# mobeets/classifying-vae-lstm

Hardware: AMD Instinct MI355X
Metric: piano-roll timesteps/sec (train) (higher is better)
Workload: dtype f32; 1 GPU; cfg3: cl_vrnn batch 256/GPU x seq_len 128, latent 2, 10 classes, 88-dim piano-roll, Adam-WN, hipGraph=True; global_batch=256, seq_len=128, parallelism=dp1

## Files before the change

### classifying-vae-lstm_amd/csrc/label_head.hip

```cpp
#include "common.h"
#include "lstm_pair_pack.h"
#include "philox.h"
#include "reduce_job.h"
#include "label_bwd_row.h"

namespace clv {

struct LabelFwdArgs {
  int B, D, C, G4;
  const float* hW;
  __device__ float* hW_out() const { return const_cast<float*>(hW); }
  const float* Ka;
  const float* ba;
  float* eps;
  struct { int on; uint32_t k0, k1, stream, step; uint64_t first; const int32_t* step_dev; } noise;
  const float* onehot;
  float prior;
  const float* Kenc_w;
  const float* benc;
  const float* Kdec_w;
  const float* bdec;
  float* wargs;
  float* W;
  float* rowloss;
  float* rb_enc;
  float* rb_dec;
};

template <int NT>
__device__ __forceinline__ void label_fwd_row(const LabelFwdArgs& a, int b, int tid, const float* s_h, float* s_wargs, float* s_w,
                                              long long oh_row = -1) {
  const int C1 = a.C - 1, NA = 2 * C1;
  __shared__ float s_eps[LH_MAXC], s_oh[LH_MAXC];
  if (tid >= NT - 64 && tid - (NT - 64) < a.C) {
    const int j = tid - (NT - 64);
    float e = 0.f;
    if (j < C1) {
      if (a.noise.on) {
        e = philox_normal_at(a.noise.first + (uint64_t)b * C1 + j, a.noise.k0, a.noise.k1, a.noise.stream,
                             a.noise.step + (a.noise.step_dev ? (uint32_t)*a.noise.step_dev : 0u));
        a.eps[(size_t)b * C1 + j] = e;
      } else {
        e = a.eps[(size_t)b * C1 + j];
      }
    }
    s_eps[j] = e;
    s_oh[j] = a.onehot ? a.onehot[(size_t)(oh_row < 0 ? b : oh_row) * a.C + j] : 0.f;
  }
  {
    __shared__ float s_part[16][2 * LH_MAXC];
    constexpr int KSL = NT / 64 < 16 ? NT / 64 : 16;
    const int col = tid & 63, sl = tid >> 6;
    if (sl < KSL) {
      float kv[(128 + KSL - 1) / KSL];
      const int cc = min(col, NA - 1);
#pragma unroll
      for (int i = 0; i < (128 + KSL - 1) / KSL; ++i) kv[i] = a.Ka[(size_t)min(sl + KSL * i, a.D - 1) * NA + cc];
      float acc = 0.f;
#pragma unroll
      for (int i = 0; i < (128 + KSL - 1) / KSL; ++i) acc = fmaf(sl + KSL * i < a.D ? s_h[sl + KSL * i] : 0.f, kv[i], acc);
      if (col < NA) s_part[sl][col] = acc;
    }
    __syncthreads();
    if (tid < NA) {
      float acc = a.ba[tid];
#pragma unroll
      for (int i = 0; i < KSL; ++i) acc += s_part[i][tid];
      s_wargs[tid] = acc;
      a.wargs[(size_t)b * NA + tid] = acc;
    }
  }
  __syncthreads();
  if (tid == 0) {
    float e[LH_MAXC];
    float S = 1.f, klw = 0.f;
    const float ep = __expf(a.prior);
    for (int j = 0; j < C1; ++j) {
      const float m = s_wargs[j], lv = s_wargs[C1 + j];
      const float sd = expf(0.5f * lv);
      e[j] = expf(m + sd * s_eps[j]);
      S += e[j];
      klw += 1.f - a.prior + lv - sd * sd / ep - m * m / ep;
    }
    e[C1] = 1.f;
    const float invS = 1.f / S;
    float qs = 0.f, wbest = -1.f, tbest = -1.f;
    int amax = 0, tmax = 0;
    for (int j = 0; j < a.C; ++j) {
      const float w = e[j] * invS;
      s_w[j] = w;
      a.W[(size_t)b * a.C + j] = w;
      qs += w + LW2;
      if (w > wbest) { wbest = w; amax = j; }
      const float tj = s_oh[j];
      if (tj > tbest) { tbest = tj; tmax = j; }
    }
    float wrec = 0.f;
    if (a.onehot)
      for (int j = 0; j < a.C; ++j) {
        const float n = (s_w[j] + LW2) / qs;
        wrec -= s_oh[j] * logf(fminf(fmaxf(n, LEPS_K), 1.f - LEPS_K));
      }
    a.rowloss[(size_t)b * 3 + 0] = -0.5f * klw;
    a.rowloss[(size_t)b * 3 + 1] = (float)C1 * wrec;
    a.rowloss[(size_t)b * 3 + 2] = (a.onehot && amax == tmax) ? 1.f : 0.f;
  }
  __syncthreads();
  for (int c = tid; c < a.G4; c += NT) {
    float e = a.benc[c], d = a.bdec[c];
    for (int j0 = 0; j0 < a.C; j0 += 8) {
      float ke[8], kd[8];
#pragma unroll
      for (int q = 0; q < 8; ++q) {
        const int j = min(j0 + q, a.C - 1);
        ke[q] = a.Kenc_w[(size_t)j * a.G4 + c];
        kd[q] = a.Kdec_w[(size_t)j * a.G4 + c];
      }
#pragma unroll
      for (int q = 0; q < 8; ++q) {
        const float w = j0 + q < a.C ? s_w[j0 + q] : 0.f;
        e = fmaf(w, ke[q], e);
        d = fmaf(w, kd[q], d);
      }
    }
    a.rb_enc[(size_t)b * a.G4 + c] = e;
    a.rb_dec[(size_t)b * a.G4 + c] = d;
  }
}

__global__ __launch_bounds__(LH_T) void vrnn_label_fwd_kernel(LabelFwdArgs a) {
  __shared__ float s_h[128], s_wargs[2 * LH_MAXC], s_w[LH_MAXC];
  const int b = blockIdx.x, tid = threadIdx.x;
  if (tid < a.D) s_h[tid] = a.hW[(size_t)b * a.D + tid];
  __syncthreads();
  label_fwd_row<LH_T>(a, b, tid, s_h, s_wargs, s_w);
}

struct LabelFwdXArgs {
  LabelFwdArgs l;
  const float* X;
  const float* Kh;
  const float* bh;
  int nx, ldx;
  PairPackArgs pack;
  const float* part; int splits;
  struct Stage {
    int on;
    const unsigned char* cur; const unsigned char* hist;
    long long cur_stride, cur_offset, hist_stride, hist_offset, row0;
    const long long* cur_table; const long long* hist_table; const long long* idx;
    const int* step_dev; int step0, period; long long cur_s, cur_o;
    float* X; float* Xh; int hist_chunk; long long hist_ld;
    const float* w_src; float* w_out;
    unsigned char* X8; unsigned char* Xh8;
  } stage;
};
__device__ __forceinline__ void label_fwd_x_block(const LabelFwdXArgs& ax, const int b, float2 (*part)[64], float* s_h, float* s_wargs,
                                                  float* s_w) {
  const LabelFwdArgs& a = ax.l;
  const int tid = threadIdx.x, lane = tid & 63;
  if (ax.pack.out) {
    for (int i = b * 1024 + tid; i < PK_TOTAL; i += a.B * 1024)
      ax.pack.out[i] = pair_pack_element(i, ax.pack.L, ax.pack.U_e, ax.pack.U_d, ax.pack.Kz, ax.pack.Wz,
                                         [](const float* p) { return *p; });
  }
  const int wave = __builtin_amdgcn_readfirstlane(tid >> 6);
  const int n2 = a.D / 2;
  const int lc = min(lane, n2 - 1);
  const float2* K2 = reinterpret_cast<const float2*>(ax.Kh);
  const float* xr = ax.X + (size_t)b * ax.ldx;
  const unsigned char* xbytes = nullptr;
  long long oh_row = -1;
  if (ax.stage.on) {
    const LabelFwdXArgs::Stage& g = ax.stage;
    long long base = 0;
    if (g.step_dev) {
      int j = (*g.step_dev - g.step0) % g.period;
      j = j < 0 ? j + g.period : j;
      base = (long long)j * g.cur_s + g.cur_o;
    }
    const long long sr = g.idx ? g.idx[base + b] : g.row0 + base + b;
    oh_row = sr;
    xbytes = g.cur + (g.cur_table ? g.cur_table[sr] : sr) * g.cur_stride + g.cur_offset;
    const unsigned char* hb = g.hist ? g.hist + (g.hist_table ? g.hist_table[sr] : sr) * g.hist_stride + g.hist_offset : nullptr;
    if (g.X8) {
      unsigned* xo8 = reinterpret_cast<unsigned*>(g.X8 + (size_t)b * ax.nx);
      unsigned* ho8 = reinterpret_cast<unsigned*>(g.Xh8 + (size_t)b * ax.nx);
      for (int c = 4 * tid; c < ax.nx; c += 4 * 1024) {
        xo8[c >> 2] = *reinterpret_cast<const unsigned*>(xbytes + c);
        if (hb) ho8[c >> 2] = *reinterpret_cast<const unsigned*>(hb + c);
      }
    } else {
      float* xo = g.X + (size_t)b * ax.ldx;
      for (int c = 4 * tid; c < ax.nx; c += 4 * 1024) {
        const unsigned v = *reinterpret_cast<const unsigned*>(xbytes + c);
        *reinterpret_cast<float4*>(xo + c) = make_float4((float)(v & 255u), (float)((v >> 8) & 255u), (float)((v >> 16) & 255u), (float)(v >> 24));
      }
      if (hb) {
        const int pieces = ax.nx / g.hist_chunk;
        for (int c = 4 * tid; c < ax.nx; c += 4 * 1024) {
          const unsigned v = *reinterpret_cast<const unsigned*>(hb + c);
          const int p = c / g.hist_chunk, w = c - p * g.hist_chunk;
          *reinterpret_cast<float4*>(g.Xh + ((size_t)b * pieces + p) * g.hist_ld + w) =
              make_float4((float)(v & 255u), (float)((v >> 8) & 255u), (float)((v >> 16) & 255u), (float)(v >> 24));
        }
      }
    }
    if (g.w_out && tid < a.C) g.w_out[(size_t)b * a.C + tid] = g.w_src[(size_t)sr * a.C + tid];
  }
  float2 acc = make_float2(0.f, 0.f);
  const int nchunk = (ax.nx + 63) / 64;
  typedef const __attribute__((address_space(1))) unsigned* gwords;
  auto xload = [&](int ch) -> unsigned {
    const int i = min(min(ch, nchunk - 1) * 64 + lane, ax.nx - 1);
    return xbytes ? ((gwords)xbytes)[i >> 2] : __builtin_bit_cast(unsigned, xr[i]);
  };
  const int xsh = 8 * (lane & 3);
  auto xval = [&](unsigned raw) { return xbytes ? (float)((raw >> xsh) & 0xffu) : __builtin_bit_cast(float, raw); };
  unsigned xa = xload(wave), xb = xload(wave + 16);
  for (int ch = wave; ch < nchunk; ch += 32) {
    const float x0 = xval(xa), x1 = xval(xb);
    const int j0 = ch * 64, j1 = (ch + 16) * 64;
    xa = xload(ch + 32); xb = xload(ch + 48);
    unsigned long long m0 = __ballot(j0 + lane < ax.nx && x0 != 0.f);
    unsigned long long m1 = __ballot(ch + 16 < nchunk && j1 + lane < ax.nx && x1 != 0.f);
    while (m0 | m1) {
      int kk[8];
      float vv[8];
#pragma unroll
      for (int q = 0; q < 8; ++q) {
        unsigned long long& m = q < 4 ? m0 : m1;
        const bool on = m != 0;
        const int bit = on ? __builtin_ctzll(m) : 0;
        m = on ? (m & (m - 1)) : 0;
        kk[q] = (q < 4 ? j0 : j1) + bit;
        const float v = __builtin_bit_cast(float, __builtin_amdgcn_readlane(__builtin_bit_cast(int, q < 4 ? x0 : x1), bit));
        vv[q] = on ? v : 0.f;
      }
      float2 kr[8];
#pragma unroll
      for (int q = 0; q < 8; ++q) kr[q] = K2[(size_t)min(kk[q], ax.nx - 1) * n2 + lc];
#pragma unroll
      for (int q = 0; q < 8; ++q) { acc.x = fmaf(vv[q], kr[q].x, acc.x); acc.y = fmaf(vv[q], kr[q].y, acc.y); }
    }
  }
  part[wave][lane] = acc;
  __syncthreads();
  if (wave == 0 && lane < n2) {
    float2 t = make_float2(ax.bh[2 * lane], ax.bh[2 * lane + 1]);
#pragma unroll
    for (int w = 0; w < 16; ++w) { t.x += part[w][lane].x; t.y += part[w][lane].y; }
    t.x = fmaxf(t.x, 0.f); t.y = fmaxf(t.y, 0.f);
    s_h[2 * lane] = t.x; s_h[2 * lane + 1] = t.y;
    float* op = a.hW_out() + (size_t)b * a.D + 2 * lane;
    op[0] = t.x; op[1] = t.y;
  }
  __syncthreads();
  label_fwd_row<1024>(a, b, tid, s_h, s_wargs, s_w, oh_row);
}

__global__ __launch_bounds__(1024) void vrnn_label_fwd_x_kernel(LabelFwdXArgs ax) {
  __shared__ float2 part[16][64];
  __shared__ float s_h[128], s_wargs[2 * LH_MAXC], s_w[LH_MAXC];
  label_fwd_x_block(ax, (int)blockIdx.x, part, s_h, s_wargs, s_w);
}

constexpr int FP_RMAX = 64;
constexpr int FP_NC = 4;
#ifndef FP_PF
#define FP_PF 4
#endif
#ifndef FP_ROUND
#define FP_ROUND 1
#endif
#ifndef FP_ABL
#define FP_ABL 0
#endif
typedef unsigned u32x4_t __attribute__((ext_vector_type(4)));
struct FrameProjArgs {
  int T, N, ldo, wgs, nset;
  const float* K[2];
  float* out[2];
};

#ifdef FRONT_STAMPS
__device__ unsigned long long g_front_wg[2048][6];
#define FRONT_STAMP(k)                                                                                               \
  do {                                                                                                               \
    __syncthreads();                                                                                                 \
    if (threadIdx.x == 0 && blockIdx.x < 2048) {                                                                     \
      unsigned long long t__;                                                                                        \
      unsigned hw__, xcc__;                                                                                          \
      asm volatile("s_memrealtime %0\n\ts_waitcnt lgkmcnt(0)" : "=s"(t__));                                          \
      asm volatile("s_getreg_b32 %0, hwreg(HW_REG_HW_ID)" : "=s"(hw__));                                             \
      asm volatile("s_getreg_b32 %0, hwreg(HW_REG_XCC_ID)" : "=s"(xcc__));                                           \
      g_front_wg[blockIdx.x][k < 2 ? k : k + 2] = t__;                                                                \
      g_front_wg[blockIdx.x][2] = hw__; g_front_wg[blockIdx.x][3] = xcc__;                                           \
    }                                                                                                                \
  } while (0)
#else
#define FRONT_STAMP(k)
#endif

__device__ __forceinline__ void frame_proj_block(const LabelFwdXArgs& ax, const FrameProjArgs& fp, const int u, float* Kl,
                                                 const unsigned char** rowp) {
  const LabelFwdXArgs::Stage& g = ax.stage;
  const int tid = threadIdx.x, lane = tid & 63;
  const int wave = __builtin_amdgcn_readfirstlane(tid >> 6);
  const int grp = u / fp.wgs, w = u - grp * fp.wgs;
  const bool second = grp >= 2;
  const int nf = ax.l.D, B = ax.l.B;
  const int nch = fp.N / 2, c0 = (grp & 1) * nch;
  const float* K = second ? fp.K[1] : fp.K[0];
  float* out = second ? fp.out[1] : fp.out[0];
  {
    const int q4 = nch / 4, nv = nf * q4;
    float4* dst = reinterpret_cast<float4*>(Kl);
    for (int i0 = tid; i0 < nv; i0 += 4 * 1024) {
      float4 v[4];
#pragma unroll
      for (int q = 0; q < 4; ++q) {
        const int e = min(i0 + q * 1024, nv - 1), k = e / q4;
        v[q] = *reinterpret_cast<const float4*>(K + (size_t)k * fp.N + c0 + 4 * (e - k * q4));
      }
#pragma unroll
      for (int q = 0; q < 4; ++q)
        if (i0 + q * 1024 < nv) dst[i0 + q * 1024] = v[q];
    }
  }
  const int nrows = w < B ? (B - w + fp.wgs - 1) / fp.wgs : 0;
  if (tid < nrows) {
    const int b = w + tid * fp.wgs;
    long long base = 0;
    if (g.step_dev) {
      int j = (*g.step_dev - g.step0) % g.period;
      j = j < 0 ? j + g.period : j;
      base = (long long)j * g.cur_s + g.cur_o;
    }
    const long long sr = g.idx ? g.idx[base + b] : g.row0 + base + b;
    rowp[tid] = second ? g.hist + (g.hist_table ? g.hist_table[sr] : sr) * g.hist_stride + g.hist_offset
                       : g.cur + (g.cur_table ? g.cur_table[sr] : sr) * g.cur_stride + g.cur_offset;
  }
  __syncthreads();
  FRONT_STAMP(2);
  const int nq = nrows * fp.T;
  if (nq == 0) return;
  const int colb = min(lane, nch / 4 - 1) * 4;
  const unsigned vo = lane < nch / 4 ? (unsigned)lane * 16u : 0x80000000u;
  const __amdgpu_buffer_rsrc_t r_out = __builtin_amdgcn_make_buffer_rsrc(out, 0, (int)((size_t)B * fp.T * fp.ldo * 4), 0x00020000);
  const int k0 = min(lane, nf - 1), k1 = min(lane + 64, nf - 1);
  const bool v0 = lane < nf, v1 = lane + 64 < nf;
  typedef const __attribute__((address_space(1))) unsigned* gwords;
  const int w0 = k0 >> 2, w1 = k1 >> 2, sh0 = 8 * (k0 & 3), sh1 = 8 * (k1 & 3), nfw = nf / 4;
  auto rowbase = [&](int r) -> gwords {
    const unsigned long long p = (unsigned long long)rowp[min(r, nrows - 1)];
    const unsigned lo = __builtin_amdgcn_readfirstlane((unsigned)p), hi = __builtin_amdgcn_readfirstlane((unsigned)(p >> 32));
    return (gwords)(((unsigned long long)hi << 32) | lo);
  };
  const gwords base0 = rowbase(0);
  auto frame = [&](gwords base, int t, unsigned& x0, unsigned& x1) {
    gwords bp = base + t * nfw;
    x0 = bp[w0]; x1 = bp[w1];
  };
  int ri = wave / fp.T, t = wave - ri * fp.T;
  int ra = ri, ta = t;
  gwords base_a = rowbase(ra);
  auto advance_a = [&]() {
    ta += 16;
    if (ta >= fp.T) {
      do { ta -= fp.T; ++ra; } while (ta >= fp.T);
      base_a = rowbase(ra);
    }
  };
  const unsigned so_step = 16u * (unsigned)fp.ldo * 4u, so_wrap = (unsigned)(fp.wgs - 1) * (unsigned)fp.T * (unsigned)fp.ldo * 4u;
  unsigned so = (unsigned)(((w + ri * fp.wgs) * fp.T + t) * fp.ldo + c0) * 4u;
  auto advance_c = [&]() {
    t += 16; so += so_step;
    while (t >= fp.T) { t -= fp.T; so += so_wrap; }
  };
  unsigned qx0[FP_PF], qx1[FP_PF];
#pragma unroll
  for (int j = 0; j < FP_PF; ++j) {
    const bool ok = wave + 16 * j < nq;
    frame(ok ? base_a : base0, ok ? ta : 0, qx0[j], qx1[j]);
    __builtin_amdgcn_raw_buffer_store_b128(u32x4_t{0u, 0u, 0u, 0u}, r_out, (int)0x80000000u, 0, 0);
    advance_a();
  }
  for (int qb = wave; qb < nq; qb += 16 * FP_PF) {
#pragma unroll
    for (int j = 0; j < FP_PF; ++j) {
      const int q = qb + 16 * j;
      const bool live = q < nq;
      const float fx0 = (float)((qx0[j] >> sh0) & 0xffu), fx1 = (float)((qx1[j] >> sh1) & 0xffu);
      const bool more = q + 16 * FP_PF < nq;
      if (FP_ABL != 3) frame(more ? base_a : base0, more ? ta : 0, qx0[j], qx1[j]);
      advance_a();
      unsigned long long m0 = __ballot(live && v0 && fx0 != 0.f), m1 = __ballot(live && v1 && fx1 != 0.f);
      float acc[FP_NC];
#pragma unroll
      for (int c = 0; c < FP_NC; ++c) acc[c] = 0.f;
      auto rounds = [&](unsigned long long m, const float fx, const int kbase) {
        if (FP_ROUND == 1) {
          while (m) {
            const int k = __builtin_ctzll(m);
            asm("s_bitset0_b64 %0, %1" : "+s"(m) : "s"(k));
            const float v = __builtin_bit_cast(float, __builtin_amdgcn_readlane(__builtin_bit_cast(int, fx), k));
            const float4 k4 = *reinterpret_cast<const float4*>(Kl + (kbase + k) * nch + colb);
            acc[0] = fmaf(v, k4.x, acc[0]); acc[1] = fmaf(v, k4.y, acc[1]); acc[2] = fmaf(v, k4.z, acc[2]); acc[3] = fmaf(v, k4.w, acc[3]);
          }
          return;
        }
        while (m) {
          float v[FP_ROUND], kv[FP_ROUND][FP_NC];
          bool on[FP_ROUND];
#pragma unroll
          for (int r = 0; r < FP_ROUND; ++r) {
            on[r] = m != 0;
            const int k = on[r] ? __builtin_ctzll(m) : 0;
            m &= m - 1;
            v[r] = __builtin_bit_cast(float, __builtin_amdgcn_readlane(__builtin_bit_cast(int, fx), k));
            const float4 k4 = *reinterpret_cast<const float4*>(Kl + (kbase + k) * nch + colb);
            kv[r][0] = k4.x; kv[r][1] = k4.y; kv[r][2] = k4.z; kv[r][3] = k4.w;
          }
#pragma unroll
          for (int r = 0; r < FP_ROUND; ++r)
#pragma unroll
            for (int c = 0; c < FP_NC; ++c) acc[c] = (r == 0 || on[r]) ? fmaf(v[r], kv[r][c], acc[c]) : acc[c];
        }
      };
      if (FP_ABL != 2) {
        rounds(m0, fx0, 0);
        rounds(m1, fx1, 64);
      } else {
        acc[0] = fx0; acc[1] = fx1;
      }
      __builtin_amdgcn_raw_buffer_store_b128(u32x4_t{__builtin_bit_cast(unsigned, acc[0]), __builtin_bit_cast(unsigned, acc[1]),
                                                      __builtin_bit_cast(unsigned, acc[2]), __builtin_bit_cast(unsigned, acc[3])},
                                             r_out, (int)((live && FP_ABL != 1) ? vo : 0x80000000u), (int)so, 0);
      advance_c();
    }
  }
}

__global__ __launch_bounds__(1024) __attribute__((amdgpu_num_sgpr(72))) void vrnn_front_kernel(LabelFwdXArgs ax, FrameProjArgs fp) {
  __shared__ float2 part[16][64];
  __shared__ float s_h[128], s_wargs[2 * LH_MAXC], s_w[LH_MAXC];
  __shared__ const unsigned char* rowp[FP_RMAX];
  extern __shared__ __attribute__((aligned(16))) float fp_kl[];
  FRONT_STAMP(0);
  if ((int)blockIdx.x < ax.l.B) label_fwd_x_block(ax, (int)blockIdx.x, part, s_h, s_wargs, s_w);
  else frame_proj_block(ax, fp, (int)blockIdx.x - ax.l.B, fp_kl, rowp);
  FRONT_STAMP(1);
}

__global__ __launch_bounds__(LH_T) void vrnn_label_fwd_parts_kernel(LabelFwdXArgs ax) {
  constexpr int NWV = LH_T / 64;
  __shared__ float2 part[NWV][64];
  __shared__ float s_h[128], s_wargs[2 * LH_MAXC], s_w[LH_MAXC];
  const LabelFwdArgs& a = ax.l;
  const int tid = threadIdx.x, lane = tid & 63;
  if (ax.pack.out) {
    for (int i = blockIdx.x * LH_T + tid; i < PK_TOTAL; i += gridDim.x * LH_T)
      ax.pack.out[i] = pair_pack_element(i, ax.pack.L, ax.pack.U_e, ax.pack.U_d, ax.pack.Kz, ax.pack.Wz,
                                         [](const float* p) { return *p; });
  }
  const int wave = __builtin_amdgcn_readfirstlane(tid >> 6);
  const int b = blockIdx.x;
  const int n2 = a.D / 2;
  const int lc = min(lane, n2 - 1);
  float2 acc = make_float2(0.f, 0.f);
  const float2* pp = reinterpret_cast<const float2*>(ax.part + (size_t)b * a.D) + lc;
  const size_t cs = (size_t)a.B * a.D / 2;
  for (int c0 = wave; c0 < ax.splits; c0 += 8 * NWV) {
    float2 v[8];
#pragma unroll
    for (int q = 0; q < 8; ++q) v[q] = pp[(size_t)min(c0 + NWV * q, ax.splits - 1) * cs];
#pragma unroll
    for (int q = 0; q < 8; ++q) {
      const float mk = c0 + NWV * q < ax.splits ? 1.f : 0.f;
      acc.x = fmaf(v[q].x, mk, acc.x); acc.y = fmaf(v[q].y, mk, acc.y);
    }
  }
  part[wave][lane] = acc;
  __syncthreads();
  if (wave == 0 && lane < n2) {
    float2 t = make_float2(ax.bh[2 * lane], ax.bh[2 * lane + 1]);
#pragma unroll
    for (int w = 0; w < NWV; ++w) { t.x += part[w][lane].x; t.y += part[w][lane].y; }
    t.x = fmaxf(t.x, 0.f); t.y = fmaxf(t.y, 0.f);
    s_h[2 * lane] = t.x; s_h[2 * lane + 1] = t.y;
    float* op = a.hW_out() + (size_t)b * a.D + 2 * lane;
    op[0] = t.x; op[1] = t.y;
  }
  __syncthreads();
  label_fwd_row<LH_T>(a, b, tid, s_h, s_wargs, s_w);
}

__global__ __launch_bounds__(LH_T) void vrnn_label_bwd_kernel(LabelBwdArgs a) {
  label_bwd_row<LH_T>(a, (int)blockIdx.x, (int)threadIdx.x);
}

}

using namespace clv;

extern "C" int clv_vrnn_label_fwd(int B, int D, int C, int G4, const float* hW, const float* Ka, const float* ba,
                                  const float* eps, const float* onehot, float prior_logvar,
                                  const float* Kenc_w, const float* benc, const float* Kdec_w, const float* bdec,
                                  float* wargs, float* W, float* rowloss, float* rb_enc, float* rb_dec, void* stream) {
  if (B <= 0 || D <= 0 || D > 128 || C < 2 || C > LH_MAXC || G4 <= 0) return CLV_EINVAL;
  if (!hW || !Ka || !ba || !eps || !Kenc_w || !benc || !Kdec_w || !bdec || !wargs || !W || !rowloss || !rb_enc || !rb_dec)
    return CLV_EINVAL;
  LabelFwdArgs a{B, D, C, G4, hW, Ka, ba, const_cast<float*>(eps), {0, 0, 0, 0, 0, 0, nullptr}, onehot, prior_logvar, Kenc_w, benc,
                 Kdec_w, bdec, wargs, W, rowloss, rb_enc, rb_dec};
  hipStream_t s = (hipStream_t)stream;
  ProfScope p("vrnn_label_fwd", s);
  hipLaunchKernelGGL(vrnn_label_fwd_kernel, dim3(B), dim3(LH_T), 0, s, a);
  return launch_status();
}

extern "C" size_t clv_vrnn_label_bwd_workspace_bytes(int B, int D, int C) {
  return (size_t)B * (D + 1) * 2 * (C - 1) * sizeof(float);
}

extern "C" int clv_vrnn_label_bwd(int B, int D, int C, int G4, const float* dzsum_enc, const float* dzsum_dec,
                                     const float* Kenc_w, const float* Kdec_w, const float* wargs, const float* eps,
                                     const float* onehot, const float* W, const float* hW, const float* Ka,
                                     float prior_logvar, float class_weight, float w_kl_weight, float inv_b,
                                     float* dwargs, float* dhW, float* dKa, float* dba, void* ws, size_t ws_bytes,
                                     clv_reduce_job* job, void* stream) {
  if (job) memset(job, 0, sizeof(*job));
  if (B <= 0 || D <= 0 || D > 128 || C < 2 || C > LH_MAXC || G4 <= 0) return CLV_EINVAL;
  if (!dzsum_enc || !dzsum_dec || !Kenc_w || !Kdec_w || !wargs || !eps || !onehot || !W || !hW || !Ka || !dwargs || !dhW)
    return CLV_EINVAL;
  const bool wg = dKa != nullptr;
  if (wg && (!dba || !ws || ws_bytes < clv_vrnn_label_bwd_workspace_bytes(B, D, C))) return CLV_EWORKSPACE;
  LabelBwdArgs a{B, D, C, G4, dzsum_enc, dzsum_dec, Kenc_w, Kdec_w, wargs, eps, onehot, W, hW, Ka,
                 prior_logvar, class_weight, w_kl_weight, inv_b, dwargs, dhW, wg ? (float*)ws : nullptr};
  hipStream_t s = (hipStream_t)stream;
  {
    ProfScope p("vrnn_label_bwd", s);
    hipLaunchKernelGGL(vrnn_label_bwd_kernel, dim3(B), dim3(LH_T), 0, s, a);
  }
  int st = launch_status();
  if (st || !wg) return st;
  ReduceJob j;
  memset(&j, 0, sizeof(j));
  const int NA = 2 * (C - 1);
  j.partial = (const float*)ws;
  j.M = D + 1; j.N = NA; j.splits = B; j.nprob = 2;
  j.alpha = 1.f; j.beta = 0.f; j.act = CLV_ACT_NONE;
  j.prob[0] = ReduceProb{dKa, NA, 0};
  j.prob[1] = ReduceProb{dba, NA, D};
  if (job && B > 1) memcpy(job, &j, sizeof(j));
  else st = launch_reduce(j, s);
  return st;
}

extern "C" int clv_vrnn_label_fwd_x_proj_supported(int B, int D, int nx, int T, int N);

static int label_fwd_x_launch(int B, int D, int C, int G4, const float* X, int ldx, int nx, const float* Kh, const float* part,
                              int splits, const clv_label_stage* stage, const float* bh, float* hW_out, const float* Ka, const float* ba,
                              float* eps, const float* onehot, float prior_logvar,
                              const float* Kenc_w, const float* benc, const float* Kdec_w, const float* bdec,
                              float* wargs, float* W, float* rowloss, float* rb_enc, float* rb_dec,
                              const clv_noise_draw* noise, const clv_pair_pack_src* pack, const clv_frame_proj* proj, void* stream) {
  if (pack && (pack->H != LH || !clv_lstm_pair_supported(pack->H, pack->L) || !pack->U_enc || !pack->U_dec || !pack->Kz ||
               !pack->Wz || !pack->pack || ((uintptr_t)pack->pack) % 16))
    return CLV_EINVAL;
  if (B <= 0 || D <= 0 || D > 128 || D % 2 != 0 || C < 2 || C > LH_MAXC || G4 <= 0) return CLV_EINVAL;
  if (part ? (splits <= 0 || ((uintptr_t)part) % 8 != 0)
           : (nx <= 0 || ldx < nx || (!X && !(stage && stage->X8)) || !Kh || ((uintptr_t)Kh) % 8 != 0)) return CLV_EINVAL;
  if (stage) {
    const clv_label_stage& g = *stage;
    if (part || !g.cur || nx % 4 || ldx % 4 || ((uintptr_t)g.cur) % 4 || g.cur_stride % 4 || g.cur_offset % 4) return CLV_EINVAL;
    if (g.hist && (((uintptr_t)g.hist) % 4 || g.hist_stride % 4 || g.hist_offset % 4)) return CLV_EINVAL;
    if (g.X8) {
      if (((uintptr_t)g.X8) % 4 || (g.hist && (!g.Xh8 || ((uintptr_t)g.Xh8) % 4))) return CLV_EINVAL;
    } else {
      if (!g.X || ((uintptr_t)g.X) % 16) return CLV_EINVAL;
      if (g.hist && (!g.Xh || g.hist_chunk <= 0 || g.hist_chunk % 4 || nx % g.hist_chunk || g.hist_ld % 4 || g.hist_ld < g.hist_chunk ||
                     ((uintptr_t)g.Xh) % 16))
        return CLV_EINVAL;
    }
    if ((g.w_out != nullptr) != (g.w_src != nullptr)) return CLV_EINVAL;
    if (g.cursor.step_dev && g.cursor.period < 1) return CLV_EINVAL;
  }
  if (!bh || !hW_out || !Ka || !ba || !eps || !Kenc_w || !benc || !Kdec_w || !bdec || !wargs || !W || !rowloss ||
      !rb_enc || !rb_dec)
    return CLV_EINVAL;
  LabelFwdXArgs a{{B, D, C, G4, hW_out, Ka, ba, eps, {0, 0, 0, 0, 0, 0, nullptr}, onehot, prior_logvar, Kenc_w, benc, Kdec_w, bdec,
                   wargs, W, rowloss, rb_enc, rb_dec}, X, Kh, bh, nx, ldx, {0, nullptr, nullptr, nullptr, nullptr, nullptr}, part, splits, {}};
  if (stage) {
    const clv_label_stage& g = *stage;
    a.stage = LabelFwdXArgs::Stage{1, g.cur, g.hist, (long long)g.cur_stride, (long long)g.cur_offset, (long long)g.hist_stride,
                                   (long long)g.hist_offset, (long long)g.row0, (const long long*)g.cur_table,
                                   (const long long*)g.hist_table, (const long long*)g.idx, g.cursor.step_dev, g.cursor.step0,
                                   g.cursor.period, (long long)g.cursor.stride, (long long)g.cursor.offset, g.X, g.Xh, g.hist_chunk,
                                   (long long)g.hist_ld, g.w_src, g.w_out, g.X8, g.Xh8};
    if (g.w_src) a.l.onehot = g.w_src;
  }
  if (pack) a.pack = PairPackArgs{pack->L, pack->U_enc, pack->U_dec, pack->Kz, pack->Wz, reinterpret_cast<float4*>(pack->pack)};
  if (noise) {
    a.l.noise.on = 1; a.l.noise.k0 = (uint32_t)noise->seed; a.l.noise.k1 = (uint32_t)(noise->seed >> 32);
    a.l.noise.stream = noise->stream; a.l.noise.step = noise->step; a.l.noise.first = noise->first;
    a.l.noise.step_dev = noise->step_dev;
  }
  hipStream_t s = (hipStream_t)stream;
  if (proj) {
    if (!clv_vrnn_label_fwd_x_proj_supported(B, D, nx, proj->T, proj->N) || !stage || !stage->X8 || part || proj->ldo < proj->N ||
        (size_t)B * proj->T * proj->ldo * 4 >= ((size_t)1 << 31) || proj->ldo % 4 || ((uintptr_t)proj->out_cur) % 16 || ((uintptr_t)proj->out_hist) % 16 ||
        !proj->K_cur || !proj->out_cur || ((uintptr_t)proj->K_cur) % 16 || (proj->K_hist && (!proj->out_hist || !stage->hist ||
        ((uintptr_t)proj->K_hist) % 16)))
      return CLV_EINVAL;
    FrameProjArgs fp;
    memset(&fp, 0, sizeof(fp));
    fp.T = proj->T; fp.N = proj->N; fp.ldo = proj->ldo; fp.nset = proj->K_hist ? 2 : 1;
    fp.K[0] = proj->K_cur; fp.out[0] = proj->out_cur; fp.K[1] = proj->K_hist; fp.out[1] = proj->out_hist;
    const int groups = 2 * fp.nset;
    int wgs = 256 / groups;
    wgs = wgs > B ? B : wgs;
    const int need = (B + FP_RMAX - 1) / FP_RMAX;
    wgs = wgs < need ? need : wgs;
    fp.wgs = wgs;
    size_t lds = (size_t)D * (proj->N / 2) * sizeof(float);
#ifdef FRONT_STAMPS
    if (const char* e = getenv("CLV_EXP_FRONT_LDS")) lds = (size_t)atoi(e);
#endif
    if (int e = clv::allow_dynamic_lds(reinterpret_cast<const void*>(vrnn_front_kernel), 64 * 1024)) return e;
    ProfScope p("vrnn_front", s);
    hipLaunchKernelGGL(vrnn_front_kernel, dim3(B + groups * wgs), dim3(1024), lds, s, a, fp);
    return launch_status();
  }
  ProfScope p("vrnn_label_fwd", s);
  if (part) hipLaunchKernelGGL(vrnn_label_fwd_parts_kernel, dim3(B), dim3(LH_T), 0, s, a);
  else hipLaunchKernelGGL(vrnn_label_fwd_x_kernel, dim3(B), dim3(1024), 0, s, a);
  return launch_status();
}

#ifdef FRONT_STAMPS
extern "C" int clv_debug_front_wg(unsigned long long* host_out) {
  return (int)hipMemcpyFromSymbol(host_out, HIP_SYMBOL(clv::g_front_wg), sizeof(unsigned long long) * 2048 * 6);
}
#endif

extern "C" int clv_vrnn_label_fwd_x_proj_supported(int B, int D, int nx, int T, int N) {
  return B >= 1 && D >= 4 && D <= 128 && D % 4 == 0 && T >= 1 && (long long)T * D == nx && N >= 8 && N % 8 == 0 && N / 2 <= 64 * clv::FP_NC &&
         (size_t)D * (N / 2) * sizeof(float) <= 64 * 1024 && (size_t)B * T * N * sizeof(float) < ((size_t)1 << 31);
}

extern "C" int clv_vrnn_label_fwd_x(int B, int D, int C, int G4, const float* X, int ldx, int nx, const float* Kh,
                                    const clv_label_stage* stage,
                                    const float* bh, float* hW_out, const float* Ka, const float* ba,
                                    float* eps, const float* onehot, float prior_logvar,
                                    const float* Kenc_w, const float* benc, const float* Kdec_w, const float* bdec,
                                    float* wargs, float* W, float* rowloss, float* rb_enc, float* rb_dec,
                                    const clv_noise_draw* noise, const clv_pair_pack_src* pack, const clv_frame_proj* proj,
                                    void* stream) {
  if (stage)
    return label_fwd_x_launch(B, D, C, G4, stage->X, ldx, nx, Kh, nullptr, 0, stage, bh, hW_out, Ka, ba, eps, stage->w_src,
                              prior_logvar, Kenc_w, benc, Kdec_w, bdec, wargs, W, rowloss, rb_enc, rb_dec, noise, pack, proj, stream);
  if (proj) return CLV_EINVAL;
  return label_fwd_x_launch(B, D, C, G4, X, ldx, nx, Kh, nullptr, 0, nullptr, bh, hW_out, Ka, ba, eps, onehot, prior_logvar, Kenc_w, benc,
                            Kdec_w, bdec, wargs, W, rowloss, rb_enc, rb_dec, noise, pack, nullptr, stream);
}

extern "C" int clv_vrnn_label_fwd_parts(int B, int D, int C, int G4, const float* part, int splits,
                                        const float* bh, float* hW_out, const float* Ka, const float* ba,
                                        float* eps, const float* onehot, float prior_logvar,
                                        const float* Kenc_w, const float* benc, const float* Kdec_w, const float* bdec,
                                        float* wargs, float* W, float* rowloss, float* rb_enc, float* rb_dec,
                                        const clv_noise_draw* noise, const clv_pair_pack_src* pack, void* stream) {
  if (!part) return CLV_EINVAL;
  return label_fwd_x_launch(B, D, C, G4, nullptr, 0, 0, nullptr, part, splits, nullptr, bh, hW_out, Ka, ba, eps, onehot, prior_logvar, Kenc_w,
                            benc, Kdec_w, bdec, wargs, W, rowloss, rb_enc, rb_dec, noise, pack, nullptr, stream);
}
```

Measured before the change: 101.5 million timesteps/s.

## Restructure sparse frame projection into per-quarter-wave nonzero compaction via LDS lists

Rewrites the piano-roll frame-projection loop so each wave handles groups of four timesteps, one per 16-lane quarter. The nonzero notes of each frame are compacted into an LDS slot list using byte-SWAR tests and DPP prefix sums, replacing the per-wave ballot/readlane loop over set bits. Each lane then accumulates three column groups of four with packed FMAs, and the prefetch depth drops from 4 to 2. The label-head scratch now aliases dynamic LDS, and the LDS request grows to hold the note lists, which lowers the supported N and adds complexity and risk in the slot indexing.

Result: no change. 103.1 million timesteps/s (median of 6 runs) (+1.5%).

```diff
diff --git a/classifying-vae-lstm_amd/csrc/label_head.hip b/classifying-vae-lstm_amd/csrc/label_head.hip
--- a/classifying-vae-lstm_amd/csrc/label_head.hip
+++ b/classifying-vae-lstm_amd/csrc/label_head.hip
@@ -267,16 +267,17 @@
 
 constexpr int FP_RMAX = 64;
 constexpr int FP_NC = 4;
+constexpr int FP_NG = 3;
+__host__ __device__ constexpr int fp_slots(int D) { return D + 4 < 128 ? D + 4 : 128; }
 #ifndef FP_PF
-#define FP_PF 4
-#endif
-#ifndef FP_ROUND
-#define FP_ROUND 1
+#define FP_PF 2
 #endif
 #ifndef FP_ABL
 #define FP_ABL 0
 #endif
 typedef unsigned u32x4_t __attribute__((ext_vector_type(4)));
+typedef float f32x2_t __attribute__((ext_vector_type(2)));
+typedef float f32x4_t __attribute__((ext_vector_type(4)));
 struct FrameProjArgs {
   int T, N, ldo, wgs, nset;
   const float* K[2];
@@ -302,8 +303,10 @@
 #define FRONT_STAMP(k)
 #endif
 
+#define FP_DPP(x, ctrl) ((unsigned)__builtin_amdgcn_update_dpp(0, (int)(x), ctrl, 0xf, 0xf, true))
+
 __device__ __forceinline__ void frame_proj_block(const LabelFwdXArgs& ax, const FrameProjArgs& fp, const int u, float* Kl,
-                                                 const unsigned char** rowp) {
+                                                 const unsigned char** rowp, unsigned short* notes) {
   const LabelFwdXArgs::Stage& g = ax.stage;
   const int tid = threadIdx.x, lane = tid & 63;
   const int wave = __builtin_amdgcn_readfirstlane(tid >> 6);
@@ -341,115 +344,134 @@
     rowp[tid] = second ? g.hist + (g.hist_table ? g.hist_table[sr] : sr) * g.hist_stride + g.hist_offset
                        : g.cur + (g.cur_table ? g.cur_table[sr] : sr) * g.cur_stride + g.cur_offset;
   }
+  const int r4 = lane >> 4, j = lane & 15;
+  const int S = fp_slots(nf);
+  unsigned short* lrow = notes + ((wave << 2) + r4) * S;
+  for (int i = j; i < S; i += 16) lrow[i] = 0;
   __syncthreads();
   FRONT_STAMP(2);
-  const int nq = nrows * fp.T;
-  if (nq == 0) return;
-  const int colb = min(lane, nch / 4 - 1) * 4;
-  const unsigned vo = lane < nch / 4 ? (unsigned)lane * 16u : 0x80000000u;
+  if (nrows == 0) return;
+  const int G = (fp.T + 3) >> 2, ng = nrows * G;
+  const int per = (ng + 15) >> 4;
+  const int g0 = wave * per, g1 = min(g0 + per, ng);
+  const int nfw = nf >> 2;
+  const int wj0 = min(j, nfw - 1), wj1 = min(j + 16, nfw - 1);
+  const bool dv0 = j < nfw, dv1 = j + 16 < nfw;
+  const unsigned kb0 = (unsigned)min(4 * j, nf - 4) << 8, kb1 = (unsigned)min(64 + 4 * j, nf - 4) << 8;
   const __amdgpu_buffer_rsrc_t r_out = __builtin_amdgcn_make_buffer_rsrc(out, 0, (int)((size_t)B * fp.T * fp.ldo * 4), 0x00020000);
-  const int k0 = min(lane, nf - 1), k1 = min(lane + 64, nf - 1);
-  const bool v0 = lane < nf, v1 = lane + 64 < nf;
+  const char* kc[FP_NG];
+  unsigned vo[FP_NG];
+#pragma unroll
+  for (int q = 0; q < FP_NG; ++q) {
+    const int col = 64 * q + FP_NC * j;
+    kc[q] = reinterpret_cast<const char*>(Kl + min(col, nch - FP_NC));
+    vo[q] = col < nch ? (unsigned)(r4 * fp.ldo + col) * 4u : 0x80000000u;
+  }
+  const unsigned pitch = (unsigned)nch * 4u, slast = (unsigned)(S - 1) * 0x01010101u;
   typedef const __attribute__((address_space(1))) unsigned* gwords;
-  const int w0 = k0 >> 2, w1 = k1 >> 2, sh0 = 8 * (k0 & 3), sh1 = 8 * (k1 & 3), nfw = nf / 4;
   auto rowbase = [&](int r) -> gwords {
     const unsigned long long p = (unsigned long long)rowp[min(r, nrows - 1)];
     const unsigned lo = __builtin_amdgcn_readfirstlane((unsigned)p), hi = __builtin_amdgcn_readfirstlane((unsigned)(p >> 32));
     return (gwords)(((unsigned long long)hi << 32) | lo);
   };
   const gwords base0 = rowbase(0);
-  auto frame = [&](gwords base, int t, unsigned& x0, unsigned& x1) {
-    gwords bp = base + t * nfw;
-    x0 = bp[w0]; x1 = bp[w1];
+  int ri = g0 / G, tg = g0 - ri * G;
+  int ra = ri, tga = tg;
+  gwords base_a = rowbase(ra);
+  auto request = [&](const bool ok, unsigned& x0, unsigned& x1) {
+    const gwords bp = ok ? base_a : base0;
+    const int t = ok ? min(4 * tga + r4, fp.T - 1) : 0;
+    x0 = bp[t * nfw + wj0]; x1 = bp[t * nfw + wj1];
+    if (++tga == G) { tga = 0; ++ra; base_a = rowbase(ra); }
   };
-  int ri = wave / fp.T, t = wave - ri * fp.T;
-  int ra = ri, ta = t;
-  gwords base_a = rowbase(ra);
-  auto advance_a = [&]() {
-    ta += 16;
-    if (ta >= fp.T) {
-      do { ta -= fp.T; ++ra; } while (ta >= fp.T);
-      base_a = rowbase(ra);
-    }
-  };
-  const unsigned so_step = 16u * (unsigned)fp.ldo * 4u, so_wrap = (unsigned)(fp.wgs - 1) * (unsigned)fp.T * (unsigned)fp.ldo * 4u;
-  unsigned so = (unsigned)(((w + ri * fp.wgs) * fp.T + t) * fp.ldo + c0) * 4u;
-  auto advance_c = [&]() {
-    t += 16; so += so_step;
-    while (t >= fp.T) { t -= fp.T; so += so_wrap; }
-  };
+  const unsigned so_step = 4u * (unsigned)fp.ldo * 4u, so_row = (unsigned)fp.wgs * (unsigned)fp.T * (unsigned)fp.ldo * 4u;
+  unsigned so0 = (unsigned)((w + ri * fp.wgs) * fp.T * fp.ldo + c0) * 4u;
   unsigned qx0[FP_PF], qx1[FP_PF];
 #pragma unroll
-  for (int j = 0; j < FP_PF; ++j) {
-    const bool ok = wave + 16 * j < nq;
-    frame(ok ? base_a : base0, ok ? ta : 0, qx0[j], qx1[j]);
-    __builtin_amdgcn_raw_buffer_store_b128(u32x4_t{0u, 0u, 0u, 0u}, r_out, (int)0x80000000u, 0, 0);
-    advance_a();
-  }
-  for (int qb = wave; qb < nq; qb += 16 * FP_PF) {
-#pragma unroll
-    for (int j = 0; j < FP_PF; ++j) {
-      const int q = qb + 16 * j;
-      const bool live = q < nq;
-      const float fx0 = (float)((qx0[j] >> sh0) & 0xffu), fx1 = (float)((qx1[j] >> sh1) & 0xffu);
-      const bool more = q + 16 * FP_PF < nq;
-      if (FP_ABL != 3) frame(more ? base_a : base0, more ? ta : 0, qx0[j], qx1[j]);
-      advance_a();
-      unsigned long long m0 = __ballot(live && v0 && fx0 != 0.f), m1 = __ballot(live && v1 && fx1 != 0.f);
-      float acc[FP_NC];
-#pragma unroll
-      for (int c = 0; c < FP_NC; ++c) acc[c] = 0.f;
-      auto rounds = [&](unsigned long long m, const float fx, const int kbase) {
-        if (FP_ROUND == 1) {
-          while (m) {
-            const int k = __builtin_ctzll(m);
-            asm("s_bitset0_b64 %0, %1" : "+s"(m) : "s"(k));
-            const float v = __builtin_bit_cast(float, __builtin_amdgcn_readlane(__builtin_bit_cast(int, fx), k));
-            const float4 k4 = *reinterpret_cast<const float4*>(Kl + (kbase + k) * nch + colb);
-            acc[0] = fmaf(v, k4.x, acc[0]); acc[1] = fmaf(v, k4.y, acc[1]); acc[2] = fmaf(v, k4.z, acc[2]); acc[3] = fmaf(v, k4.w, acc[3]);
+  for (int s = 0; s < FP_PF; ++s) {
+    request(g0 + s < g1, qx0[s], qx1[s]);
+#pragma unroll
+    for (int q = 0; q < FP_NG; ++q) __builtin_amdgcn_raw_buffer_store_b128(u32x4_t{0u, 0u, 0u, 0u}, r_out, (int)0x80000000u, 0, 0);
+  }
+  for (int gb = g0; gb < g1; gb += FP_PF) {
+#pragma unroll
+    for (int s = 0; s < FP_PF; ++s) {
+      const int gi = gb + s;
+      const bool fv = gi < g1 && 4 * tg + r4 < fp.T;
+      const unsigned a0 = fv && dv0 ? qx0[s] : 0u, a1 = fv && dv1 ? qx1[s] : 0u;
+      if (FP_ABL != 3) request(gi + FP_PF < g1, qx0[s], qx1[s]);
+      f32x2_t acc[FP_NG][2];
+#pragma unroll
+      for (int q = 0; q < FP_NG; ++q) acc[q][0] = acc[q][1] = f32x2_t{0.f, 0.f};
+      if (FP_ABL != 2) {
+        const unsigned y0 = (((a0 & 0x7f7f7f7fu) + 0x7f7f7f7fu) | a0) & 0x80808080u;
+        const unsigned y1 = (((a1 & 0x7f7f7f7fu) + 0x7f7f7f7fu) | a1) & 0x80808080u;
+        const unsigned own = (unsigned)__builtin_popcount(y0) | ((unsigned)__builtin_popcount(y1) << 16);
+        unsigned inc = own;
+        inc += FP_DPP(inc, 0x111); inc += FP_DPP(inc, 0x112); inc += FP_DPP(inc, 0x114); inc += FP_DPP(inc, 0x118);
+        const unsigned tot = FP_DPP(inc, 0x15f), ex = inc - own;
+        const unsigned cnt = (tot & 0xffffu) + (tot >> 16);
+        auto put = [&](const unsigned a, const unsigned y, const unsigned rank, const unsigned kb) {
+          const unsigned z = y ^ 0x80808080u, zm = (z - (z >> 7)) & slast;
+#pragma unroll
+          for (int p = 0; p < 4; ++p) {
+            const unsigned below = p ? (unsigned)__builtin_popcount(y & ((1u << (8 * p)) - 1u)) : 0u;
+            const unsigned slot = max(rank + below, (zm >> (8 * p)) & 0xffu);
+            lrow[slot] = (unsigned short)((kb + ((unsigned)p << 8)) | ((a >> (8 * p)) & 0xffu));
           }
-          return;
+        };
+        put(a0, y0, ex & 0xffffu, kb0);
+        put(a1, y1, (tot & 0xffffu) + (ex >> 16), kb1);
+        __builtin_amdgcn_wave_barrier();
+        const int c01 = max(__builtin_amdgcn_readlane((int)cnt, 0), __builtin_amdgcn_readlane((int)cnt, 16));
+        const int c23 = max(__builtin_amdgcn_readlane((int)cnt, 32), __builtin_amdgcn_readlane((int)cnt, 48));
+        const int nr = max(c01, c23);
+        unsigned e = *(const volatile __attribute__((address_space(3))) unsigned short*)lrow;
+        float vn = (float)(e & 0xffu);
+        unsigned ko = __umul24(e >> 8, pitch);
+#pragma nounroll
+        for (int i = 0; i < nr; ++i) {
+          e = lrow[i + 1];
+          f32x2_t vv;
+          vv.x = vv.y = (unsigned)i < cnt ? vn : 0.f;
+          asm("" : "+v"(vv));
+          f32x4_t k4[FP_NG];
+#pragma unroll
+          for (int q = 0; q < FP_NG; ++q) k4[q] = *reinterpret_cast<const f32x4_t*>(kc[q] + ko);
+          vn = (float)(e & 0xffu);
+          ko = __umul24(e >> 8, pitch);
+#pragma unroll
+          for (int q = 0; q < FP_NG; ++q) {
+            acc[q][0] = __builtin_elementwise_fma(vv, k4[q].xy, acc[q][0]);
+            acc[q][1] = __builtin_elementwise_fma(vv, k4[q].zw, acc[q][1]);
+          }
         }
-        while (m) {
-          float v[FP_ROUND], kv[FP_ROUND][FP_NC];
-          bool on[FP_ROUND];
-#pragma unroll
-          for (int r = 0; r < FP_ROUND; ++r) {
-            on[r] = m != 0;
-            const int k = on[r] ? __builtin_ctzll(m) : 0;
-            m &= m - 1;
-            v[r] = __builtin_bit_cast(float, __builtin_amdgcn_readlane(__builtin_bit_cast(int, fx), k));
-            const float4 k4 = *reinterpret_cast<const float4*>(Kl + (kbase + k) * nch + colb);
-            kv[r][0] = k4.x; kv[r][1] = k4.y; kv[r][2] = k4.z; kv[r][3] = k4.w;
-          }
-#pragma unroll
-          for (int r = 0; r < FP_ROUND; ++r)
-#pragma unroll
-            for (int c = 0; c < FP_NC; ++c) acc[c] = (r == 0 || on[r]) ? fmaf(v[r], kv[r][c], acc[c]) : acc[c];
-        }
-      };
-      if (FP_ABL != 2) {
-        rounds(m0, fx0, 0);
-        rounds(m1, fx1, 64);
       } else {
-        acc[0] = fx0; acc[1] = fx1;
-      }
-      __builtin_amdgcn_raw_buffer_store_b128(u32x4_t{__builtin_bit_cast(unsigned, acc[0]), __builtin_bit_cast(unsigned, acc[1]),
-                                                      __builtin_bit_cast(unsigned, acc[2]), __builtin_bit_cast(unsigned, acc[3])},
-                                             r_out, (int)((live && FP_ABL != 1) ? vo : 0x80000000u), (int)so, 0);
-      advance_c();
+        acc[0][0] = f32x2_t{__builtin_bit_cast(float, a0), __builtin_bit_cast(float, a1)};
+      }
+      const unsigned so = so0 + (unsigned)tg * so_step;
+      unsigned vq[FP_NG];
+#pragma unroll
+      for (int q = 0; q < FP_NG; ++q) vq[q] = (fv && FP_ABL != 1) ? vo[q] : 0x80000000u;
+#pragma unroll
+      for (int q = 0; q < FP_NG; ++q) {
+        __builtin_amdgcn_raw_buffer_store_b128(__builtin_bit_cast(u32x4_t, __builtin_shufflevector(acc[q][0], acc[q][1], 0, 1, 2, 3)),
+                                               r_out, (int)vq[q], (int)so, 0);
+        asm volatile("s_nop 1");
+        __builtin_amdgcn_sched_barrier(0);
+      }
+      if (++tg == G) { tg = 0; so0 += so_row; }
     }
   }
 }
 
 __global__ __launch_bounds__(1024) __attribute__((amdgpu_num_sgpr(72))) void vrnn_front_kernel(LabelFwdXArgs ax, FrameProjArgs fp) {
-  __shared__ float2 part[16][64];
   __shared__ float s_h[128], s_wargs[2 * LH_MAXC], s_w[LH_MAXC];
   __shared__ const unsigned char* rowp[FP_RMAX];
   extern __shared__ __attribute__((aligned(16))) float fp_kl[];
   FRONT_STAMP(0);
-  if ((int)blockIdx.x < ax.l.B) label_fwd_x_block(ax, (int)blockIdx.x, part, s_h, s_wargs, s_w);
-  else frame_proj_block(ax, fp, (int)blockIdx.x - ax.l.B, fp_kl, rowp);
+  if ((int)blockIdx.x < ax.l.B) label_fwd_x_block(ax, (int)blockIdx.x, reinterpret_cast<float2(*)[64]>(fp_kl), s_h, s_wargs, s_w);
+  else frame_proj_block(ax, fp, (int)blockIdx.x - ax.l.B, fp_kl, rowp, reinterpret_cast<unsigned short*>(fp_kl + ax.l.D * (fp.N / 2)));
   FRONT_STAMP(1);
 }
 
@@ -623,11 +645,12 @@
     const int need = (B + FP_RMAX - 1) / FP_RMAX;
     wgs = wgs < need ? need : wgs;
     fp.wgs = wgs;
-    size_t lds = (size_t)D * (proj->N / 2) * sizeof(float);
+    size_t lds = (size_t)D * (proj->N / 2) * sizeof(float) + (size_t)64 * fp_slots(D) * sizeof(unsigned short) + 16;
+    lds = lds < 16 * 64 * sizeof(float2) ? 16 * 64 * sizeof(float2) : lds;
 #ifdef FRONT_STAMPS
     if (const char* e = getenv("CLV_EXP_FRONT_LDS")) lds = (size_t)atoi(e);
 #endif
-    if (int e = clv::allow_dynamic_lds(reinterpret_cast<const void*>(vrnn_front_kernel), 64 * 1024)) return e;
+    if (int e = clv::allow_dynamic_lds(reinterpret_cast<const void*>(vrnn_front_kernel), 64 * 1024 + 64 * 128 * 2 + 16)) return e;
     ProfScope p("vrnn_front", s);
     hipLaunchKernelGGL(vrnn_front_kernel, dim3(B + groups * wgs), dim3(1024), lds, s, a, fp);
     return launch_status();
@@ -645,7 +668,7 @@
 #endif
 
 extern "C" int clv_vrnn_label_fwd_x_proj_supported(int B, int D, int nx, int T, int N) {
-  return B >= 1 && D >= 4 && D <= 128 && D % 4 == 0 && T >= 1 && (long long)T * D == nx && N >= 8 && N % 8 == 0 && N / 2 <= 64 * clv::FP_NC &&
+  return B >= 1 && D >= 4 && D <= 128 && D % 4 == 0 && T >= 1 && (long long)T * D == nx && N >= 8 && N % 8 == 0 && N / 2 <= 16 * clv::FP_NC * clv::FP_NG &&
          (size_t)D * (N / 2) * sizeof(float) <= 64 * 1024 && (size_t)B * T * N * sizeof(float) < ((size_t)1 << 31);
 }
 
```
